# ShampooWang/SpeechCLIP_plus

Measured on AMD Instinct MI355X. Metric: utterances/sec (train step), higher is better.
Workload: dtype bf16; 1 GPU; Parallel SpeechCLIP base train step (HuBERT-base frozen fwd + weighted sum + CLS attention-pool head fwd/bwd + InfoNCE fwd/bwd + Adam), 64 utt/GPU x 10 s (L=160000, T=499), CLIP image embeddings given; global_batch=64, per_gpu_batch=64, audio_samples=160000, frames=499, parallelism=dp1

## Files before the change

speechclip_plus_amd/csrc/clspool.hip:

```cpp
#include "sc_common.h"

namespace {

constexpr int MAXH = 16;

template <int NH>
__device__ __forceinline__ float wave_sum_multi(float (&v)[NH], int lane, int& which) {
    int n = NH, off = 32;
    which = 0;
#pragma unroll
    for (int round = 0; round < 6; ++round) {
        if (n > 1) {
            const bool hi = (lane & off) != 0;
            const int half = n >> 1;
#pragma unroll
            for (int i = 0; i < NH / 2; ++i) {
                if (i < half) {
                    const float keep = hi ? v[i + half] : v[i];
                    const float send = hi ? v[i] : v[i + half];
                    v[i] = keep + __shfl_xor(send, off);
                }
            }
            which = which * 2 + (hi ? 1 : 0);
            n = half;
// ... 58 lines not shown
        }
    }
}

template <int NH>
__global__ __launch_bounds__(256) void cls_pool_fwd_kernel(const uint16_t* __restrict__ X,
                                                           const float* __restrict__ scores,
                                                           const int32_t* __restrict__ len, float* __restrict__ p,
                                                           float* __restrict__ m, int R, int D, int H,
                                                           const float* __restrict__ mult, float* __restrict__ psum) {
    extern __shared__ float sm[];
    float* ps = sm;
    float* red = sm + H * R;
    const int b = blockIdx.y, d0 = blockIdx.x * 64;
    const int lane = threadIdx.x & 63, wave = threadIdx.x >> 6;
    const int n = max(1, min(len[b], R));
    for (int h = wave; h < H; h += 4) {
        const float* sr = scores + ((int64_t)b * H + h) * R;
        float mx = -INFINITY;
        for (int s = lane; s < n; s += 64) mx = fmaxf(mx, sr[s]);
        mx = wave_max(mx);
        float sum = 0.f;
        for (int s = lane; s < n; s += 64) {
            const float e = __expf(sr[s] - mx);
            ps[h * R + s] = e;
            sum += e;
        }
        sum = wave_sum(sum);
        const float inv = 1.0f / sum;
        float kept = 0.f;
        for (int s = lane; s < R; s += 64) {
            const float v = s < n ? ps[h * R + s] * inv : 0.f;
            const float w = mult ? v * mult[((int64_t)b * H + h) * R + s] : v;
            ps[h * R + s] = w;
            kept += w;
            if (blockIdx.x == 0) p[((int64_t)b * H + h) * R + s] = v;
        }
        if (psum) {
            kept = wave_sum(kept);
            if (blockIdx.x == 0 && lane == 0) psum[(int64_t)b * H + h] = kept;
        }
    }
    __syncthreads();
    float acc[NH][8];
#pragma unroll
    for (int h = 0; h < NH; ++h)
#pragma unroll
        for (int e = 0; e < 8; ++e) acc[h][e] = 0.f;
    const int cchunk = lane & 7, rsub = lane >> 3;
    const uint16_t* xc = X + (int64_t)b * R * D + d0 + cchunk * 8;
    for (int s = wave * 8 + rsub; s < n; s += 32) {
        const uint4 u = *(const uint4*)(xc + (int64_t)s * D);
        const float x[8] = {bflo(u.x), bfhi(u.x), bflo(u.y), bfhi(u.y), bflo(u.z), bfhi(u.z), bflo(u.w), bfhi(u.w)};
#pragma unroll
        for (int h = 0; h < NH; ++h) {
            const float w = ps[h * R + s];
#pragma unroll
            for (int e = 0; e < 8; ++e) acc[h][e] = fmaf(w, x[e], acc[h][e]);
        }
    }
#pragma unroll
    for (int h = 0; h < NH; ++h)
#pragma unroll
        for (int e = 0; e < 8; ++e) {
            float v = acc[h][e];
            v += __shfl_xor(v, 8);
            v += __shfl_xor(v, 16);
            v += __shfl_xor(v, 32);
            if (rsub == 0) red[(wave * H + h) * 64 + cchunk * 8 + e] = v;
        }
    __syncthreads();
    for (int i = threadIdx.x; i < H * 64; i += 256) {
        const int h = i >> 6, d = i & 63;
        const float v = (red[(0 * H + h) * 64 + d] + red[(1 * H + h) * 64 + d]) +
                        (red[(2 * H + h) * 64 + d] + red[(3 * H + h) * 64 + d]);
        m[((int64_t)b * H + h) * D + d0 + d] = v;
    }
}

template <int NH>
__global__ __launch_bounds__(256) void cls_pool_bwd_kernel(const uint16_t* __restrict__ X,
                                                           const float* __restrict__ p,
                                                           const float* __restrict__ dp,
                                                           const float* __restrict__ dm,
                                                           const float* __restrict__ a,
                                                           const int32_t* __restrict__ len, float* __restrict__ dX,
                                                           float* __restrict__ da_partial, int R, int D, int H,
                                                           const float* __restrict__ mult, const float* __restrict__ cbias) {
    extern __shared__ float sm[];
    float* ps = sm;
    float* dss = sm + H * R;
    float* red = sm + 2 * H * R;
    const int b = blockIdx.y, d0 = blockIdx.x * 64;
    const int lane = threadIdx.x & 63, wave = threadIdx.x >> 6;
    const int n = max(1, min(len[b], R));
    for (int h = wave; h < H; h += 4) {
        const float* pr = p + ((int64_t)b * H + h) * R;
        const float* dpr = dp + ((int64_t)b * H + h) * R;
        const float* mr = mult ? mult + ((int64_t)b * H + h) * R : nullptr;
        const float cb = cbias ? cbias[(int64_t)b * H + h] : 0.f;
        auto dpe = [&](int s) { return cbias ? (dpr[s] + cb) * (mr ? mr[s] : 1.f) : dpr[s]; };
        float dot = 0.f;
        for (int s = lane; s < n; s += 64) dot += pr[s] * dpe(s);
        dot = wave_sum(dot);
        for (int s = lane; s < R; s += 64) {
            const float pv = s < n ? pr[s] : 0.f;
            ps[h * R + s] = mr ? pv * mr[s] : pv;
            dss[h * R + s] = s < n ? pv * (dpe(s) - dot) : 0.f;
        }
    }
    __syncthreads();
    const int cchunk = lane & 15, rsub = lane >> 4, c0 = d0 + cchunk * 4;
    f32x4 dmv[NH], av[NH], acc[NH];
#pragma unroll
    for (int h = 0; h < NH; ++h) {
        dmv[h] = *(const f32x4*)(dm + ((int64_t)b * H + h) * D + c0);
        av[h] = *(const f32x4*)(a + (int64_t)h * D + c0);
        acc[h] = f32x4{0.f, 0.f, 0.f, 0.f};
    }
    const uint16_t* xc = X + (int64_t)b * R * D + c0;
    float* gx = dX + (int64_t)b * R * D + c0;
    for (int s = wave * 4 + rsub; s < R; s += 16) {
        f32x4 g = {0.f, 0.f, 0.f, 0.f};
        if (s < n) {
            const uint2 u = *(const uint2*)(xc + (int64_t)s * D);
            const f32x4 x = {bflo(u.x), bfhi(u.x), bflo(u.y), bfhi(u.y)};
#pragma unroll
            for (int h = 0; h < NH; ++h) {
                const float dsv = dss[h * R + s], pw = ps[h * R + s];
                g += pw * dmv[h] + dsv * av[h];
                acc[h] += dsv * x;
            }
        }
        *(f32x4*)(gx + (int64_t)s * D) = g;
    }
#pragma unroll
    for (int h = 0; h < NH; ++h)
#pragma unroll
        for (int e = 0; e < 4; ++e) {
            float v = acc[h][e];
            v += __shfl_xor(v, 16);
            v += __shfl_xor(v, 32);
            if (rsub == 0) red[(wave * H + h) * 64 + cchunk * 4 + e] = v;
        }
    __syncthreads();
    for (int i = threadIdx.x; i < H * 64; i += 256) {
        const int h = i >> 6, d = i & 63;
        const float v = (red[(0 * H + h) * 64 + d] + red[(1 * H + h) * 64 + d]) +
                        (red[(2 * H + h) * 64 + d] + red[(3 * H + h) * 64 + d]);
        da_partial[((int64_t)b * H + h) * D + d0 + d] = v;
    }
}

}

extern "C" int sc_cls_scores(const sc_bf16* X, const float* vec, int64_t vec_bstride, float* scores, int32_t B,
                             int32_t R, int32_t D, int32_t H, void* stream) {
    SC_CHECK(X && vec && scores, "sc_cls_scores: null pointer");
    SC_CHECK(D % 4 == 0 && ((uintptr_t)X % 8) == 0 && ((uintptr_t)vec % 16) == 0 && vec_bstride % 4 == 0,
             "sc_cls_scores: alignment");
    SC_CHECK(D <= 1024, "sc_cls_scores: D=%d must be <= 1024", D);
    dim3 grid((R + 63) / 64, B);
    hipStream_t s = (hipStream_t)stream;
    const int nch = (D / 4 + 63) / 64;
#define SC_CS(NH, NC) hipLaunchKernelGGL((cls_scores_kernel<NH, NC>), grid, dim3(256), 0, s, X, vec, vec_bstride, scores, R, D, H, h0)
#define SC_CS_H(NH)                                                        \
    do {                                                                   \
        if (nch <= 1) SC_CS(NH, 1); else if (nch == 2) SC_CS(NH, 2); else if (nch == 3) SC_CS(NH, 3); else SC_CS(NH, 4); \
    } while (0)
    int h0 = 0;
    switch (H) {
        case 1: SC_CS_H(1); break;
        case 2: SC_CS_H(2); break;
        case 4: SC_CS_H(4); break;
        case 8: SC_CS_H(8); break;
        case 16:
            SC_CS_H(8);
            h0 = 8;
            SC_CS_H(8);
            break;
        default: sc_set_error("sc_cls_scores: H=%d not in {1,2,4,8,16}", H); return -1;
    }
#undef SC_CS_H
#undef SC_CS
    SC_LAUNCH_CHECK();
    return 0;
}

extern "C" int sc_cls_pool_fwd(const sc_bf16* X, const float* scores, const int32_t* len, float* p, float* m,
                               int32_t B, int32_t R, int32_t D, int32_t H, const float* mult, float* psum, void* stream) {
    SC_CHECK(X && scores && len && p && m, "sc_cls_pool_fwd: null pointer");
    SC_CHECK(D % 64 == 0 && H >= 1 && H <= MAXH && ((uintptr_t)X % 16) == 0, "sc_cls_pool_fwd: D %% 64, H <= 16, 16-byte aligned X required (D=%d H=%d)", D, H);
    const size_t lds = (size_t)(H * R + 4 * H * 64) * sizeof(float);
    SC_CHECK(lds <= 64 * 1024, "sc_cls_pool_fwd: H*R too large for LDS");
    #define SC_CPF(NH) hipLaunchKernelGGL(cls_pool_fwd_kernel<NH>, dim3(D / 64, B), dim3(256), lds, (hipStream_t)stream, X, scores, len, p, m, R, D, H, mult, psum)
    switch (H) {
        case 1: SC_CPF(1); break;
        case 2: SC_CPF(2); break;
        case 4: SC_CPF(4); break;
        case 8: SC_CPF(8); break;
        case 16: SC_CPF(16); break;
        default: sc_set_error("sc_cls_pool_fwd: H=%d not in {1,2,4,8,16}", H); return -1;
    }
#undef SC_CPF
    SC_LAUNCH_CHECK();
    return 0;
}

extern "C" int sc_cls_pool_bwd(const sc_bf16* X, const float* p, const float* dp, const float* dm, const float* a,
                               const int32_t* len, float* dX, float* da_partial, int32_t B, int32_t R, int32_t D,
                               int32_t H, const float* mult, const float* cbias, void* stream) {
    SC_CHECK(X && p && dp && dm && a && len && dX && da_partial, "sc_cls_pool_bwd: null pointer");
    SC_CHECK(D % 64 == 0 && H >= 1 && H <= MAXH, "sc_cls_pool_bwd: D %% 64, H <= 16 required");
    SC_CHECK(((uintptr_t)X % 8) == 0 && ((uintptr_t)dX % 16) == 0 && ((uintptr_t)dm % 16) == 0 && ((uintptr_t)a % 16) == 0, "sc_cls_pool_bwd: alignment");
    const size_t lds = (size_t)(2 * H * R + 4 * H * 64) * sizeof(float);
    SC_CHECK(lds <= 64 * 1024, "sc_cls_pool_bwd: H*R too large for LDS");
    #define SC_CPB(NH) hipLaunchKernelGGL(cls_pool_bwd_kernel<NH>, dim3(D / 64, B), dim3(256), lds, (hipStream_t)stream, X, p, dp, dm, a, len, dX, da_partial, R, D, H, mult, cbias)
    switch (H) {
        case 1: SC_CPB(1); break;
        case 2: SC_CPB(2); break;
        case 4: SC_CPB(4); break;
        case 8: SC_CPB(8); break;
        case 16: SC_CPB(16); break;
        default: sc_set_error("sc_cls_pool_bwd: H=%d not in {1,2,4,8,16}", H); return -1;
    }
#undef SC_CPB
    SC_LAUNCH_CHECK();
    return 0;
}
```

speechclip_plus_amd/csrc/rowops.hip:

```cpp
#include "sc_common.h"

namespace {

template <int NCH>
__global__ __launch_bounds__(256) void layernorm_kernel(const uint16_t* __restrict__ x, int64_t ldx,
                                                        const float* __restrict__ gamma,
                                                        const float* __restrict__ beta, uint16_t* __restrict__ y,
                                                        int64_t ldy, int64_t rows, int D, float eps, int act) {
    const int lane = threadIdx.x & 63;
    const int64_t row = (int64_t)blockIdx.x * 4 + (threadIdx.x >> 6);
    if (row >= rows) return;
    const int nchunks = D >> 2;
    float v[NCH][4];
    float sum = 0.f;
    const uint16_t* xr = x + row * ldx;
#pragma unroll
    for (int i = 0; i < NCH; ++i) {
        const int ch = lane + i * 64;
        if (ch < nchunks) {
            const uint2 u = *(const uint2*)(xr + ch * 4);
            v[i][0] = bflo(u.x); v[i][1] = bfhi(u.x); v[i][2] = bflo(u.y); v[i][3] = bfhi(u.y);
            sum += (v[i][0] + v[i][1]) + (v[i][2] + v[i][3]);
        } else {
            v[i][0] = v[i][1] = v[i][2] = v[i][3] = 0.f;
// ... 388 lines not shown
                load_row_norm<NE>(h + n * plane + m.src * D, lane, nchunks, D, 1e-5f, xh);
                const float wn = w[n];
#pragma unroll
                for (int i = 0; i < NE; ++i)
#pragma unroll
                    for (int j = 0; j < 8; ++j) acc[i][j] += wn * xh[i][j];
            }
        }
#pragma unroll
        for (int i = 0; i < NE; ++i) {
            const int ch = lane + i * 64;
            if (ch < nchunks) {
                uint4 o;
                o.x = pack2bf(acc[i][0], acc[i][1]); o.y = pack2bf(acc[i][2], acc[i][3]);
                o.z = pack2bf(acc[i][4], acc[i][5]); o.w = pack2bf(acc[i][6], acc[i][7]);
                *(uint4*)(out + m.out * D + ch * 8) = o;
            }
        }
    }
}

template <int NE, typename GT, typename Rows>
__global__ __launch_bounds__(256) void wsum_norm_bwd_kernel(const uint16_t* __restrict__ h, const GT* __restrict__ g, int NL,
                                                            float* __restrict__ dw_partial, Rows rows, int D, int row_off) {
    __shared__ float red[4][32];
    const int lane = threadIdx.x & 63, wave = threadIdx.x >> 6;
    const int nchunks = D >> 3;
    const int64_t count = rows.count(), plane = rows.plane(D);
    float accn[32];
#pragma unroll
    for (int n = 0; n < 32; ++n) accn[n] = 0.f;
    for (int64_t row = (int64_t)blockIdx.x * 4 + wave; row < count; row += (int64_t)gridDim.x * 4) {
        const RowRef m = rows.at(row, row_off);
        if (!m.live) continue;
        float gv[NE][8];
#pragma unroll
        for (int i = 0; i < NE; ++i) {
            const int ch = lane + i * 64;
            if (ch < nchunks) {
                f32x4 g0, g1;
                load_g8(g + m.out * D + ch * 8, g0, g1);
                gv[i][0] = g0[0]; gv[i][1] = g0[1]; gv[i][2] = g0[2]; gv[i][3] = g0[3];
                gv[i][4] = g1[0]; gv[i][5] = g1[1]; gv[i][6] = g1[2]; gv[i][7] = g1[3];
            } else {
#pragma unroll
                for (int j = 0; j < 8; ++j) gv[i][j] = 0.f;
            }
        }
        float xr[NE][8];
        load_row_norm<NE>(h + (int64_t)(NL - 1) * plane + m.src * D, lane, nchunks, D, 1e-5f, xr);
#pragma unroll
        for (int n = 0; n < 31; ++n) {
            if (n < NL - 1) {
                float xh[NE][8];
                load_row_norm<NE>(h + n * plane + m.src * D, lane, nchunks, D, 1e-5f, xh);
                float d = 0.f;
#pragma unroll
                for (int i = 0; i < NE; ++i)
#pragma unroll
                    for (int j = 0; j < 8; ++j) d += gv[i][j] * (xh[i][j] - xr[i][j]);
                accn[n] += d;
            }
        }
    }
#pragma unroll
    for (int n = 0; n < 32; ++n) {
        const float s = wave_sum(accn[n]);
        if (lane == 0) red[wave][n] = s;
    }
    __syncthreads();
    if (threadIdx.x < NL)
        dw_partial[(int64_t)blockIdx.x * NL + threadIdx.x] =
            (red[0][threadIdx.x] + red[1][threadIdx.x]) + (red[2][threadIdx.x] + red[3][threadIdx.x]);
}

__global__ __launch_bounds__(256) void posconv_prep_kernel(const uint16_t* __restrict__ x,
                                                           const int32_t* __restrict__ valid_len,
                                                           uint16_t* __restrict__ xz, uint16_t* __restrict__ xg,
                                                           int B, int R, int D, int G, int halo) {
    const int Dg = D / G;
    const int cpg = Dg >> 3;
    const int64_t chunks_per_row = D >> 3;
    const int64_t total = (int64_t)B * R * chunks_per_row;
    const int Rp = R + 2 * halo;
    for (int64_t q = (int64_t)blockIdx.x * blockDim.x + threadIdx.x; q < total; q += (int64_t)gridDim.x * blockDim.x) {
        const int64_t row = q / chunks_per_row;
        const int cc = (int)(q % chunks_per_row);
        const int b = (int)(row / R), t = (int)(row % R);
        uint4 u = make_uint4(0, 0, 0, 0);
        if (t < valid_len[b]) u = *(const uint4*)(x + row * D + cc * 8);
        *(uint4*)(xz + row * D + cc * 8) = u;
        const int g = cc / cpg, cg = cc % cpg;
        *(uint4*)(xg + (((int64_t)g * B + b) * Rp + halo + t) * Dg + cg * 8) = u;
    }
}


template <int NLT>
__global__ __launch_bounds__(256) void wsum_fwd_seg_fixed_kernel(const uint16_t* __restrict__ h, const float* __restrict__ w,
                                                                 uint16_t* __restrict__ out, const int32_t* __restrict__ row0, int Rout,
                                                                 int D, int row_off, int64_t plane) {
    const int cpr = D >> 3;
    const int idx = blockIdx.x * 256 + threadIdx.x;
    if (idx >= Rout * cpr) return;
    const int b = blockIdx.y;
    const int s = idx / cpr, cc = idx - s * cpr, t = s - row_off;
    const int r0 = row0[b], pitch = row0[b + 1] - r0;
    float acc[8] = {0, 0, 0, 0, 0, 0, 0, 0};
    if (t >= 0 && t < pitch) {
        const uint16_t* src = h + (int64_t)(r0 + t) * D + cc * 8;
        uint4 u[NLT];
#pragma unroll
        for (int n = 0; n < NLT; ++n) u[n] = *(const uint4*)(src + n * plane);
#pragma unroll
        for (int n = 0; n < NLT; ++n) {
            const float wn = w[n];
            acc[0] += wn * bflo(u[n].x); acc[1] += wn * bfhi(u[n].x); acc[2] += wn * bflo(u[n].y); acc[3] += wn * bfhi(u[n].y);
            acc[4] += wn * bflo(u[n].z); acc[5] += wn * bfhi(u[n].z); acc[6] += wn * bflo(u[n].w); acc[7] += wn * bfhi(u[n].w);
        }
    }
    uint4 o;
    o.x = pack2bf(acc[0], acc[1]); o.y = pack2bf(acc[2], acc[3]);
    o.z = pack2bf(acc[4], acc[5]); o.w = pack2bf(acc[6], acc[7]);
    *(uint4*)(out + ((int64_t)b * Rout + s) * D + cc * 8) = o;
}

template <int NLT, typename GT>
__global__ __launch_bounds__(256) void wsum_bwd_seg_fixed_kernel(const uint16_t* __restrict__ h, const GT* __restrict__ g,
                                                                 float* __restrict__ dw_partial, const int32_t* __restrict__ row0, int B, int Rout,
                                                                 int D, int row_off, int64_t plane) {
    __shared__ float red[4][32];
    const uint32_t cpr = (uint32_t)D >> 3, total = (uint32_t)B * (uint32_t)Rout * cpr, step = gridDim.x * 256u;
    float acc[NLT - 1];
#pragma unroll
    for (int n = 0; n < NLT - 1; ++n) acc[n] = 0.f;
    for (uint32_t q = blockIdx.x * 256u + threadIdx.x; q < total; q += step) {
        const uint32_t orow = q / cpr, cc = q - orow * cpr;
        const uint32_t b = orow / (uint32_t)Rout;
        const int t = (int)(orow - b * (uint32_t)Rout) - row_off;
        const int r0 = row0[b], pitch = row0[b + 1] - r0;
        if (t < 0 || t >= pitch) continue;
        f32x4 g0, g1;
        load_g8(g + (int64_t)orow * D + cc * 8, g0, g1);
        const uint16_t* src = h + (int64_t)(r0 + t) * D + cc * 8;
        const uint4 r = *(const uint4*)(src + (int64_t)(NLT - 1) * plane);
        uint4 u[NLT - 1];
#pragma unroll
        for (int n = 0; n < NLT - 1; ++n) u[n] = *(const uint4*)(src + n * plane);
#pragma unroll
        for (int n = 0; n < NLT - 1; ++n)
            acc[n] += g0[0] * (bflo(u[n].x) - bflo(r.x)) + g0[1] * (bfhi(u[n].x) - bfhi(r.x)) + g0[2] * (bflo(u[n].y) - bflo(r.y)) +
                      g0[3] * (bfhi(u[n].y) - bfhi(r.y)) + g1[0] * (bflo(u[n].z) - bflo(r.z)) + g1[1] * (bfhi(u[n].z) - bfhi(r.z)) +
                      g1[2] * (bflo(u[n].w) - bflo(r.w)) + g1[3] * (bfhi(u[n].w) - bfhi(r.w));
    }
    const int lane = threadIdx.x & 63, wave = threadIdx.x >> 6;
#pragma unroll
    for (int n = 0; n < NLT - 1; ++n) {
        const float sn = wave_sum(acc[n]);
        if (lane == 0) red[wave][n] = sn;
    }
    if (lane == 0) red[wave][NLT - 1] = 0.f;
    __syncthreads();
    if (threadIdx.x < NLT)
        dw_partial[(int64_t)blockIdx.x * NLT + threadIdx.x] =
            (red[0][threadIdx.x] + red[1][threadIdx.x]) + (red[2][threadIdx.x] + red[3][threadIdx.x]);
}

__global__ __launch_bounds__(256) void posconv_prep_seg_kernel(const uint16_t* __restrict__ x, const int32_t* __restrict__ valid_len,
                                                               uint16_t* __restrict__ xz, uint16_t* __restrict__ xg,
                                                               const int32_t* __restrict__ chunk, int rows, int B, int D, int G, int halo) {
    const int Dg = D / G;
    const int cpg = Dg >> 3;
    const int64_t chunks_per_row = D >> 3;
    const int64_t total = (int64_t)rows * chunks_per_row;
    const int64_t slab_rows = (int64_t)rows + 2 * halo * B;
    for (int64_t q = (int64_t)blockIdx.x * blockDim.x + threadIdx.x; q < total; q += (int64_t)gridDim.x * blockDim.x) {
        const int row = (int)(q / chunks_per_row);
        const int cc = (int)(q % chunks_per_row);
        const int4 sg = *(const int4*)(chunk + 4 * (row >> 3));
        const int t = row - sg.x, pitch = sg.y, b = sg.z;
        uint4 u = make_uint4(0, 0, 0, 0);
        if (t < valid_len[b]) u = *(const uint4*)(x + (int64_t)row * D + cc * 8);
        *(uint4*)(xz + (int64_t)row * D + cc * 8) = u;
        const int g = cc / cpg, cg = cc % cpg;
        uint16_t* slab = xg + ((int64_t)g * slab_rows + sg.x + 2 * halo * b) * Dg + cg * 8;
        *(uint4*)(slab + (int64_t)(halo + t) * Dg) = u;
        const uint4 z = make_uint4(0, 0, 0, 0);
        for (int v = t; v < halo; v += pitch) {
            *(uint4*)(slab + (int64_t)v * Dg) = z;
            *(uint4*)(slab + (int64_t)(halo + pitch + v) * Dg) = z;
        }
    }
}

}

extern "C" int sc_layernorm_bf16(const sc_bf16* x, int64_t ldx, const float* gamma, const float* beta, sc_bf16* y,
                                 int64_t ldy, int64_t rows, int32_t D, float eps, int32_t act, void* stream) {
    SC_CHECK(x && gamma && beta && y, "sc_layernorm_bf16: null pointer");
    SC_CHECK(D > 0 && D % 4 == 0 && D <= 1024, "sc_layernorm_bf16: D=%d must be a multiple of 4, <= 1024", D);
    SC_CHECK(ldx % 4 == 0 && ldy % 4 == 0 && rows > 0, "sc_layernorm_bf16: bad ld/rows");
    SC_CHECK(((uintptr_t)x % 8) == 0 && ((uintptr_t)y % 8) == 0 && ((uintptr_t)gamma % 16) == 0 &&
                 ((uintptr_t)beta % 16) == 0, "sc_layernorm_bf16: alignment");
    hipStream_t s = (hipStream_t)stream;
    if (D % 8 == 0 && ldx % 8 == 0 && ldy % 8 == 0 && ((uintptr_t)x % 16) == 0 && ((uintptr_t)y % 16) == 0) {
        dim3 grid8((unsigned)((rows + 7) / 8));
        const int nch8 = (D / 8 + 31) / 32;
        if (nch8 <= 2) hipLaunchKernelGGL(layernorm16_kernel<2>, grid8, dim3(256), 0, s, x, ldx, gamma, beta, y, ldy, rows, D, eps, act);
        else if (nch8 == 3) hipLaunchKernelGGL(layernorm16_kernel<3>, grid8, dim3(256), 0, s, x, ldx, gamma, beta, y, ldy, rows, D, eps, act);
        else hipLaunchKernelGGL(layernorm16_kernel<4>, grid8, dim3(256), 0, s, x, ldx, gamma, beta, y, ldy, rows, D, eps, act);
        SC_LAUNCH_CHECK();
        return 0;
    }
    dim3 grid((unsigned)((rows + 3) / 4));
    const int nch = (D / 4 + 63) / 64;
    if (nch <= 2) hipLaunchKernelGGL(layernorm_kernel<2>, grid, dim3(256), 0, s, x, ldx, gamma, beta, y, ldy, rows, D, eps, act);
    else if (nch == 3) hipLaunchKernelGGL(layernorm_kernel<3>, grid, dim3(256), 0, s, x, ldx, gamma, beta, y, ldy, rows, D, eps, act);
    else hipLaunchKernelGGL(layernorm_kernel<4>, grid, dim3(256), 0, s, x, ldx, gamma, beta, y, ldy, rows, D, eps, act);
    SC_LAUNCH_CHECK();
    return 0;
}

namespace {

template <typename Rows>
int wsum_fwd_launch(const uint16_t* h, const float* w, int NL, uint16_t* out, const Rows& rows, int D, int row_off, bool normalize, int grid,
                    hipStream_t s) {
    if (!normalize) hipLaunchKernelGGL(wsum_fwd_kernel<Rows>, dim3(grid), dim3(256), 0, s, h, w, NL, out, rows, D, row_off);
    else if (D <= 512) hipLaunchKernelGGL((wsum_norm_fwd_kernel<1, Rows>), dim3(grid), dim3(256), 0, s, h, w, NL, out, rows, D, row_off);
    else hipLaunchKernelGGL((wsum_norm_fwd_kernel<2, Rows>), dim3(grid), dim3(256), 0, s, h, w, NL, out, rows, D, row_off);
    SC_LAUNCH_CHECK();
    return 0;
}

template <typename Rows>
int wsum_bwd_launch(const uint16_t* h, const void* gv, int NL, float* dw_partial, int nblk, const Rows& rows, int D, int row_off, int flags,
                    hipStream_t s) {
    const bool normalize = flags & 1, g16 = flags & 2;
    const float* g = (const float*)gv;
    const uint16_t* gh = (const uint16_t*)gv;
    if (!normalize) {
        if (g16) hipLaunchKernelGGL((wsum_bwd_kernel<uint16_t, Rows>), dim3(nblk), dim3(256), 0, s, h, gh, NL, dw_partial, rows, D, row_off);
        else hipLaunchKernelGGL((wsum_bwd_kernel<float, Rows>), dim3(nblk), dim3(256), 0, s, h, g, NL, dw_partial, rows, D, row_off);
    } else if (D <= 512) {
        if (g16) hipLaunchKernelGGL((wsum_norm_bwd_kernel<1, uint16_t, Rows>), dim3(nblk), dim3(256), 0, s, h, gh, NL, dw_partial, rows, D, row_off);
        else hipLaunchKernelGGL((wsum_norm_bwd_kernel<1, float, Rows>), dim3(nblk), dim3(256), 0, s, h, g, NL, dw_partial, rows, D, row_off);
    } else {
        if (g16) hipLaunchKernelGGL((wsum_norm_bwd_kernel<2, uint16_t, Rows>), dim3(nblk), dim3(256), 0, s, h, gh, NL, dw_partial, rows, D, row_off);
        else hipLaunchKernelGGL((wsum_norm_bwd_kernel<2, float, Rows>), dim3(nblk), dim3(256), 0, s, h, g, NL, dw_partial, rows, D, row_off);
    }
    SC_LAUNCH_CHECK();
    return 0;
}

template int wsum_fwd_launch(const uint16_t*, const float*, int, uint16_t*, const UniformRows&, int, int, bool, int, hipStream_t);
template int wsum_bwd_launch(const uint16_t*, const void*, int, float*, int, const UniformRows&, int, int, int, hipStream_t);

}

extern "C" int sc_wsum_fwd(const sc_bf16* h, const float* w, int32_t NL, sc_bf16* out, const sc_segments* seg, int32_t B, int32_t R,
                           int32_t D, int32_t row_off, int32_t normalize, void* stream) {
    SC_CHECK(h && w && out && (!seg || seg->row0), "sc_wsum_fwd: null pointer");
    SC_CHECK(NL >= 1 && NL <= 32 && D % 8 == 0 && row_off >= 0 && row_off < R && (!seg || (seg->B > 0 && seg->rows > 0)), "sc_wsum_fwd: bad NL/D/row_off");
    SC_CHECK(!seg || B == seg->B, "sc_wsum_fwd: B=%d against seg->B=%d", B, seg->B);
    if (normalize) SC_CHECK(D <= 1024, "sc_wsum_fwd: normalised variant needs D <= 1024 (got %d)", D);
    hipStream_t s = (hipStream_t)stream;
    const int64_t plane = seg ? (int64_t)seg->rows * D : 0;
    if (seg && !normalize && (NL == 13 || NL == 25) && (int64_t)R * (D / 8) < (1ll << 30) && B <= 65535 && !sc_option(5)) {
        const dim3 g2((unsigned)(((int64_t)R * (D / 8) + 255) / 256), (unsigned)B);
        if (NL == 13) hipLaunchKernelGGL(wsum_fwd_seg_fixed_kernel<13>, g2, dim3(256), 0, s, h, w, out, seg->row0, R, D, row_off, plane);
        else hipLaunchKernelGGL(wsum_fwd_seg_fixed_kernel<25>, g2, dim3(256), 0, s, h, w, out, seg->row0, R, D, row_off, plane);
        SC_LAUNCH_CHECK();
        return 0;
    }
    const int64_t rows = (int64_t)B * R, total = rows * (D / 8);
    const int grid = normalize ? (int)((rows + 3) / 4 < 4096 ? (rows + 3) / 4 : 4096) : (int)((total + 255) / 256 < 2048 ? (total + 255) / 256 : 2048);
    return seg ? wsum_fwd_launch(h, w, NL, out, SegRows{seg->row0, B, R, plane}, D, row_off, normalize, grid, s)
               : wsum_fwd_launch(h, w, NL, out, UniformRows{B, R}, D, row_off, normalize, grid, s);
}

extern "C" int sc_wsum_bwd(const sc_bf16* h, const void* gv, int32_t NL, float* dw_partial, int32_t nblk, const sc_segments* seg, int32_t B,
                           int32_t R, int32_t D, int32_t row_off, int32_t flags, void* stream) {
    SC_CHECK(h && gv && dw_partial && (!seg || seg->row0), "sc_wsum_bwd: null pointer");
    SC_CHECK(((uintptr_t)gv % 16) == 0, "sc_wsum_bwd: g must be 16-byte aligned");
    const bool normalize = flags & 1, g16 = flags & 2;
    SC_CHECK(NL >= 1 && NL <= 32 && D % 8 == 0 && nblk >= 1 && row_off >= 0 && row_off < R && (!seg || (seg->B > 0 && seg->rows > 0)), "sc_wsum_bwd: bad args");
    SC_CHECK(!seg || B == seg->B, "sc_wsum_bwd: B=%d against seg->B=%d", B, seg->B);
    if (normalize) SC_CHECK(D <= 1024, "sc_wsum_bwd: normalised variant needs D <= 1024 (got %d)", D);
    hipStream_t s = (hipStream_t)stream;
    if (!seg) return wsum_bwd_launch(h, gv, NL, dw_partial, nblk, UniformRows{B, R}, D, row_off, flags, s);
    const int64_t plane = (int64_t)seg->rows * D;
    if (!normalize && (NL == 13 || NL == 25) && (int64_t)B * R * (D / 8) < (1ll << 31) && !sc_option(5)) {
        const float* g = (const float*)gv;
        const uint16_t* gh = (const uint16_t*)gv;
        if (NL == 13) {
            if (g16) hipLaunchKernelGGL((wsum_bwd_seg_fixed_kernel<13, uint16_t>), dim3(nblk), dim3(256), 0, s, h, gh, dw_partial, seg->row0, B, R, D, row_off, plane);
            else hipLaunchKernelGGL((wsum_bwd_seg_fixed_kernel<13, float>), dim3(nblk), dim3(256), 0, s, h, g, dw_partial, seg->row0, B, R, D, row_off, plane);
        } else {
            if (g16) hipLaunchKernelGGL((wsum_bwd_seg_fixed_kernel<25, uint16_t>), dim3(nblk), dim3(256), 0, s, h, gh, dw_partial, seg->row0, B, R, D, row_off, plane);
            else hipLaunchKernelGGL((wsum_bwd_seg_fixed_kernel<25, float>), dim3(nblk), dim3(256), 0, s, h, g, dw_partial, seg->row0, B, R, D, row_off, plane);
        }
        SC_LAUNCH_CHECK();
        return 0;
    }
    return wsum_bwd_launch(h, gv, NL, dw_partial, nblk, SegRows{seg->row0, B, R, plane}, D, row_off, flags, s);
}

extern "C" int sc_wsum_lazy_fwd(const sc_bf16* h, const float* w, int32_t NL, sc_bf16* out, int32_t B, int32_t R, int32_t D,
                                int32_t row_off, const float* stats, const float* gamma, const float* beta, int32_t first_lazy,
                                int32_t ns, float eps, void* stream) {
    SC_CHECK(h && w && out && stats && gamma && beta, "sc_wsum_lazy_fwd: null pointer");
    SC_CHECK(NL >= 1 && NL <= 32 && D % 8 == 0 && row_off >= 0 && row_off < R && ns >= 1 && ns <= 8 && first_lazy >= 0 && eps > 0.f,
             "sc_wsum_lazy_fwd: bad NL / D / row_off / strips");
    const LazyLn z{stats, gamma, beta, first_lazy, ns, eps};
    const int64_t total = (int64_t)B * R * (D / 8);
    const int grid = (int)((total + 255) / 256 < 2048 ? (total + 255) / 256 : 2048);
    hipLaunchKernelGGL(wsum_lazy_fwd_kernel, dim3(grid), dim3(256), 0, (hipStream_t)stream, h, w, NL, out, B, R, D, row_off, z);
    SC_LAUNCH_CHECK();
    return 0;
}

extern "C" int sc_wsum_lazy_bwd(const sc_bf16* h, const float* g, int32_t NL, float* dw_partial, int32_t nblk, int32_t B, int32_t R,
                                int32_t D, int32_t row_off, const float* stats, const float* gamma, const float* beta,
                                int32_t first_lazy, int32_t ns, float eps, void* stream) {
    SC_CHECK(h && g && dw_partial && stats && gamma && beta, "sc_wsum_lazy_bwd: null pointer");
    SC_CHECK(NL >= 1 && NL <= 32 && D % 8 == 0 && nblk >= 1 && row_off >= 0 && row_off < R && ns >= 1 && ns <= 8 && eps > 0.f,
             "sc_wsum_lazy_bwd: bad args");
    const LazyLn z{stats, gamma, beta, first_lazy, ns, eps};
    hipLaunchKernelGGL(wsum_lazy_bwd_kernel, dim3(nblk), dim3(256), 0, (hipStream_t)stream, h, g, NL, dw_partial, B, R, D, row_off, z);
    SC_LAUNCH_CHECK();
    return 0;
}

extern "C" int sc_posconv_prep(const sc_bf16* x, const int32_t* valid_len, sc_bf16* xz, sc_bf16* xg, const sc_segments* seg, int32_t B,
                               int32_t R, int32_t D, int32_t G, int32_t halo, void* stream) {
    SC_CHECK(x && valid_len && xz && xg && (!seg || seg->chunk), "sc_posconv_prep: null pointer");
    if (seg) {
        SC_CHECK(G > 0 && D % G == 0 && (D / G) % 8 == 0 && seg->rows > 0 && seg->rows % SC_SEG_ROWS == 0 && seg->B > 0 && halo > 0,
                 "sc_posconv_prep: D/G=%d must be a multiple of 8, rows a multiple of 8", D / G);
        SC_CHECK(((uintptr_t)seg->chunk % 16) == 0, "sc_posconv_prep: chunk table must be 16-byte aligned");
    } else {
        SC_CHECK(G > 0 && D % G == 0 && (D / G) % 8 == 0, "sc_posconv_prep: D/G=%d must be a multiple of 8", D / G);
    }
    const int64_t total = (seg ? (int64_t)seg->rows : (int64_t)B * R) * (D / 8);
    const int grid = (int)((total + 255) / 256 < 4096 ? (total + 255) / 256 : 4096);
    if (seg)
        hipLaunchKernelGGL(posconv_prep_seg_kernel, dim3(grid), dim3(256), 0, (hipStream_t)stream, x, valid_len, xz, xg, seg->chunk, seg->rows, seg->B, D, G, halo);
    else
        hipLaunchKernelGGL(posconv_prep_kernel, dim3(grid), dim3(256), 0, (hipStream_t)stream, x, valid_len, xz, xg, B, R, D, G, halo);
    SC_LAUNCH_CHECK();
    return 0;
}
```

Baseline: 5641 utterances/s.

## Add hand-scheduled variants of CLS pooling and layer weighted-sum kernels

Adds new variants of the CLS score, pooling forward and backward kernels and of the segmented weighted-sum forward and backward kernels, selected by default unless option 4 is set. The new kernels use 32-bit offsets, scalar base pointers, LDS-staged weight tables, two rows per iteration and asm register ties that force load and FMA ordering, while reproducing the original kernels' rounding order. The aim is lower address arithmetic, better memory-level parallelism and fewer wasted loads in these bandwidth-bound passes. This adds a large amount of fragile code that depends on specific head and layer counts and on exact compiler rounding behaviour.

```diff
diff --git a/speechclip_plus_amd/csrc/clspool.hip b/speechclip_plus_amd/csrc/clspool.hip
--- a/speechclip_plus_amd/csrc/clspool.hip
+++ b/speechclip_plus_amd/csrc/clspool.hip
@@ -234,6 +234,315 @@
     }
 }
 
+
+
+__device__ __forceinline__ float dot4(int first, float x0, float x1, float x2, float x3, const f32x4& v) {
+#pragma clang fp contract(off)
+    float t = first ? x1 * v[1] : x0 * v[0];
+    t = first ? fmaf(x0, v[0], t) : fmaf(x1, v[1], t);
+    t = fmaf(x2, v[2], t);
+    return fmaf(x3, v[3], t);
+}
+
+template <int NH>
+__device__ __forceinline__ float wave_sum_multi_late(float (&v)[NH], int lane, int& which) {
+    auto shfl_xor = [&](float x, int off) { return __int_as_float(__builtin_amdgcn_ds_bpermute((lane ^ off) << 2, __float_as_int(x))); };
+    int n = NH, off = 32;
+    which = 0;
+#pragma unroll
+    for (int round = 0; round < 6; ++round) {
+        if (n > 1) {
+            const bool hi = (lane & off) != 0;
+            const int half = n >> 1;
+#pragma unroll
+            for (int i = 0; i < NH / 2; ++i) {
+                if (i < half) {
+                    const float keep = hi ? v[i + half] : v[i];
+                    const float send = hi ? v[i] : v[i + half];
+                    v[i] = keep + shfl_xor(send, off);
+                }
+            }
+            which = which * 2 + (hi ? 1 : 0);
+            n = half;
+        } else {
+            v[0] += shfl_xor(v[0], off);
+        }
+        off >>= 1;
+    }
+    return v[0];
+}
+
+template <int NH, int NCH>
+__global__ __launch_bounds__(256) void cls_scores_co_kernel(const uint16_t* __restrict__ X, const float* __restrict__ vec, int64_t vec_bstride,
+                                                            float* __restrict__ scores, int R, int Htot, int h0) {
+    constexpr int D = 256 * NCH;
+    const int b = blockIdx.y;
+    const int lane = threadIdx.x & 63, wave = threadIdx.x >> 6;
+    const float* vb = vec + (int64_t)b * vec_bstride + (int64_t)h0 * D;
+    __shared__ f32x4 vs[NH * 64 * NCH];
+    for (int i = threadIdx.x; i < NH * 64 * NCH; i += 256) vs[i] = *(const f32x4*)(vb + (int64_t)i * 4);
+    __syncthreads();
+    constexpr int ROWS = 64, RPW = ROWS / 4;
+    static_assert(NH == 8, "dot4's table of roundings is the 8-head kernels'");
+    constexpr unsigned kMulFirst1 = NCH == 1 ? 0xaau : 0x56u;
+    const int s0 = blockIdx.x * ROWS + wave * RPW;
+    const char* xb = (const char*)X + (int64_t)b * R * D * 2;
+#pragma unroll 1
+    for (int g = 0; g < RPW; g += 2) {
+        int vo = lane;
+        asm volatile("" : "+v"(vo));
+        uint2 u0[NCH], u1[NCH];
+        {
+            const uint32_t o0 = (uint32_t)min(s0 + g, R - 1) * (uint32_t)(D * 2) + (uint32_t)vo * 8u;
+            const uint32_t o1 = (uint32_t)min(s0 + g + 1, R - 1) * (uint32_t)(D * 2) + (uint32_t)vo * 8u;
+#pragma unroll
+            for (int c = 0; c < NCH; ++c) {
+                u0[c] = *(const uint2*)(xb + o0 + 512 * c);
+                u1[c] = *(const uint2*)(xb + o1 + 512 * c);
+            }
+        }
+        float acc0[NH], acc1[NH];
+#pragma unroll
+        for (int h = 0; h < NH; ++h) acc0[h] = acc1[h] = 0.f;
+#pragma unroll
+        for (int c = 0; c < NCH; ++c) {
+            if (c > 0) asm("" : "+v"(u0[c].x), "+v"(u0[c].y), "+v"(u1[c].x), "+v"(u1[c].y) : "v"(acc0[NH - 1]), "v"(acc1[NH - 1]));
+            const float x0 = bflo(u0[c].x), x1 = bfhi(u0[c].x), x2 = bflo(u0[c].y), x3 = bfhi(u0[c].y);
+            const float y0 = bflo(u1[c].x), y1 = bfhi(u1[c].x), y2 = bflo(u1[c].y), y3 = bfhi(u1[c].y);
+#pragma unroll
+            for (int h = 0; h < NH; ++h) {
+                int vk = vo;
+                const int k2 = c * NH + h - 2;
+                if (k2 >= 0) asm("" : "+v"(vk) : "v"(acc0[k2 % NH]), "v"(acc1[k2 % NH]));
+                const f32x4 v = vs[h * (64 * NCH) + 64 * c + vk];
+                acc0[h] += dot4((kMulFirst1 >> h) & 1, x0, x1, x2, x3, v);
+                acc1[h] += dot4((kMulFirst1 >> h) & 1, y0, y1, y2, y3, v);
+            }
+        }
+        constexpr int LOWMASK = 63 >> 3;
+        int h, ln = vo;
+        asm volatile("" : "+v"(ln) : "v"(acc0[NH - 1]), "v"(acc1[NH - 1]));
+        const float t0 = wave_sum_multi_late<NH>(acc0, ln, h);
+        if ((ln & LOWMASK) == 0 && s0 + g < R) scores[((int64_t)b * Htot + h0 + h) * R + s0 + g] = t0;
+        const float t1 = wave_sum_multi_late<NH>(acc1, ln, h);
+        if ((ln & LOWMASK) == 0 && s0 + g + 1 < R) scores[((int64_t)b * Htot + h0 + h) * R + s0 + g + 1] = t1;
+    }
+}
+
+template <int NH>
+__global__ __launch_bounds__(256) void cls_pool_fwd_co_kernel(const uint16_t* __restrict__ X, const float* __restrict__ scores,
+                                                              const int32_t* __restrict__ len, float* __restrict__ p, float* __restrict__ m, int R,
+                                                              int D, int H, const float* __restrict__ mult, float* __restrict__ psum) {
+    extern __shared__ float sm[];
+    float* ps = sm;
+    float* red = sm + H * R;
+    const int b = blockIdx.y, d0 = blockIdx.x * 64;
+    const int lane = threadIdx.x & 63, wave = threadIdx.x >> 6;
+    const int n = max(1, min(len[b], R));
+    for (int h = wave; h < H; h += 4) {
+        const float* sr = scores + ((int64_t)b * H + h) * R;
+        float mx = -INFINITY;
+        for (int s = lane; s < n; s += 64) mx = fmaxf(mx, sr[s]);
+        mx = wave_max(mx);
+        float sum = 0.f;
+        for (int s = lane; s < n; s += 64) {
+            const float e = __expf(sr[s] - mx);
+            ps[h * R + s] = e;
+            sum += e;
+        }
+        sum = wave_sum(sum);
+        const float inv = 1.0f / sum;
+        float kept = 0.f;
+        for (int s = lane; s < R; s += 64) {
+            const float v = s < n ? ps[h * R + s] * inv : 0.f;
+            const float w = mult ? v * mult[((int64_t)b * H + h) * R + s] : v;
+            ps[h * R + s] = w;
+            kept += w;
+            if (blockIdx.x == 0) p[((int64_t)b * H + h) * R + s] = v;
+        }
+        if (psum) {
+            kept = wave_sum(kept);
+            if (blockIdx.x == 0 && lane == 0) psum[(int64_t)b * H + h] = kept;
+        }
+    }
+    __syncthreads();
+    constexpr int HG = NH <= 4 ? NH : NH / 2;
+    const int cchunk = lane & 7, rsub = lane >> 3;
+    const uint16_t* xc = X + (int64_t)b * R * D + d0 + cchunk * 8;
+#pragma unroll 1
+    for (int hg = 0; hg < NH; hg += HG) {
+        float acc[HG][8];
+#pragma unroll
+        for (int h = 0; h < HG; ++h)
+#pragma unroll
+            for (int e = 0; e < 8; ++e) acc[h][e] = 0.f;
+        const float* pg = ps + hg * R;
+#pragma unroll 1
+        for (int s = wave * 8 + rsub; s < n; s += 32) {
+            const uint4 u = *(const uint4*)(xc + (int64_t)s * D);
+            const float x[8] = {bflo(u.x), bfhi(u.x), bflo(u.y), bfhi(u.y), bflo(u.z), bfhi(u.z), bflo(u.w), bfhi(u.w)};
+#pragma unroll
+            for (int h = 0; h < HG; ++h) {
+                int sw = s;
+                if (h > 0) asm("" : "+v"(sw) : "v"(acc[h - 1][7]));
+                const float w = pg[h * R + sw];
+#pragma unroll
+                for (int e = 0; e < 8; ++e) acc[h][e] = fmaf(w, x[e], acc[h][e]);
+            }
+        }
+#pragma unroll
+        for (int h = 0; h < HG; ++h)
+#pragma unroll
+            for (int e = 0; e < 8; ++e) {
+                float v = acc[h][e];
+                v += __shfl_xor(v, 8);
+                v += __shfl_xor(v, 16);
+                v += __shfl_xor(v, 32);
+                if (rsub == 0) red[(wave * H + hg + h) * 64 + cchunk * 8 + e] = v;
+            }
+    }
+    __syncthreads();
+    for (int i = threadIdx.x; i < H * 64; i += 256) {
+        const int h = i >> 6, d = i & 63;
+        const float v = (red[(0 * H + h) * 64 + d] + red[(1 * H + h) * 64 + d]) +
+                        (red[(2 * H + h) * 64 + d] + red[(3 * H + h) * 64 + d]);
+        m[((int64_t)b * H + h) * D + d0 + d] = v;
+    }
+}
+
+template <typename T>
+__device__ __forceinline__ T* uniform_ptr(T* p) {
+    const uint64_t v = (uint64_t)p;
+    const uint32_t lo = __builtin_amdgcn_readfirstlane((uint32_t)v), hi = __builtin_amdgcn_readfirstlane((uint32_t)(v >> 32));
+    return (T*)(((uint64_t)hi << 32) | lo);
+}
+
+template <int NH>
+__global__ __launch_bounds__(256) void cls_pool_bwd_co_kernel(const uint16_t* __restrict__ X, const float* __restrict__ p,
+                                                              const float* __restrict__ dp, const float* __restrict__ dm,
+                                                              const float* __restrict__ a, const int32_t* __restrict__ len,
+                                                              float* __restrict__ dX, float* __restrict__ da_partial, int R, int D, int H,
+                                                              const float* __restrict__ mult, const float* __restrict__ cbias) {
+#pragma clang fp contract(off)
+    static_assert(NH == 8, "the roundings spelled out below are those of cls_pool_bwd_kernel<8> as compiled");
+    constexpr int TS = 128;
+    __shared__ f32x4 dms[NH][16], as[NH][16];
+    __shared__ f32x2 wt[NH][TS];
+    __shared__ float red[4 * NH * 64];
+    __shared__ float dots[NH];
+    const int b = blockIdx.y, d0 = blockIdx.x * 64;
+    const int lane = threadIdx.x & 63, wave = threadIdx.x >> 6;
+    const int n = max(1, min(len[b], R));
+    const int uwave = __builtin_amdgcn_readfirstlane(wave);
+    auto dpe = [&](const float* dpr, const float* mr, float cb, int s) { return cbias ? (dpr[s] + cb) * (mr ? mr[s] : 1.f) : dpr[s]; };
+    for (int h = uwave; h < NH; h += 4) {
+        const float* pr = p + ((int64_t)b * H + h) * R;
+        const float* dpr = dp + ((int64_t)b * H + h) * R;
+        const float* mr = mult ? mult + ((int64_t)b * H + h) * R : nullptr;
+        const float cb = cbias ? cbias[(int64_t)b * H + h] : 0.f;
+        float dot = 0.f;
+        for (int s = lane; s < n; s += 64) dot = fmaf(pr[s], dpe(dpr, mr, cb, s), dot);
+        dot = wave_sum(dot);
+        if (lane == 0) dots[h] = dot;
+    }
+    for (int i = threadIdx.x; i < NH * 16; i += 256) {
+        const int h = i >> 4, cq = i & 15;
+        dms[h][cq] = *(const f32x4*)(dm + (uint32_t)((b * H + h) * D + d0 + cq * 4));
+        as[h][cq] = *(const f32x4*)(a + (uint32_t)(h * D + d0 + cq * 4));
+    }
+    f32x4 acc[NH];
+#pragma unroll
+    for (int h = 0; h < NH; ++h)
+#pragma unroll
+        for (int e = 0; e < 4; ++e) {
+            float z = 0.f;
+            asm volatile("" : "+v"(z));
+            acc[h][e] = z;
+        }
+    const char* xb = (const char*)X + (int64_t)b * R * D * 2;
+    char* gb = (char*)dX + (int64_t)b * R * D * 4;
+    xb = uniform_ptr(xb);
+    gb = uniform_ptr(gb);
+    typedef uint32_t u32x2 __attribute__((ext_vector_type(2)));
+#pragma unroll 1
+    for (int t0 = 0; t0 < R; t0 += TS) {
+        const int t1 = min(R, t0 + TS);
+        __syncthreads();
+        for (int h = uwave; h < NH; h += 4) {
+            const float* pr = p + ((int64_t)b * H + h) * R;
+            const float* dpr = dp + ((int64_t)b * H + h) * R;
+            const float* mr = mult ? mult + ((int64_t)b * H + h) * R : nullptr;
+            const float cb = cbias ? cbias[(int64_t)b * H + h] : 0.f;
+            const float dot = dots[h];
+            int fl = threadIdx.x;
+            asm volatile("" : "+v"(fl));
+            for (int s = t0 + (fl & 63); s < t1; s += 64) {
+                const float pv = s < n ? pr[s] : 0.f;
+                f32x2 t;
+                t.x = mr ? pv * mr[s] : pv;
+                t.y = s < n ? pv * (dpe(dpr, mr, cb, s) - dot) : 0.f;
+                wt[h][s - t0] = t;
+            }
+        }
+        __syncthreads();
+        int tid = threadIdx.x;
+        asm volatile("" : "+v"(tid));
+        const int cq0 = tid & 15, co0 = d0 + cq0 * 4;
+#pragma unroll 1
+        for (int s = t0 + (tid >> 4); s < t1; s += 16) {
+            f32x4 g = {0.f, 0.f, 0.f, 0.f};
+            if (s < n) {
+                int cq = cq0;
+                asm volatile("" : "+v"(cq));
+                const u32x2 u = *(const __attribute__((address_space(1))) u32x2*)((const __attribute__((address_space(1))) char*)xb + ((uint32_t)s * (uint32_t)D + (uint32_t)co0) * 2u);
+                const f32x4 x = {bflo(u.x), bfhi(u.x), bflo(u.y), bfhi(u.y)};
+                float tie1 = 0.f, tie1b = 0.f;
+#pragma unroll
+                for (int h = 0; h < NH; ++h) {
+                    int ch = cq, sh = s - t0;
+                    if (h >= 1) asm("" : "+v"(ch), "+v"(sh) : "v"(tie1), "v"(tie1b), "v"(acc[h - 1][1]), "v"(acc[h - 1][3]));
+                    else asm("" : "+v"(ch), "+v"(sh) : "v"(x[1]), "v"(x[3]));
+                    const f32x2 t = wt[h][sh];
+                    const float dsv = t.y, pw = t.x;
+#pragma unroll
+                    for (int e2 = 0; e2 < 2; ++e2) {
+                        const int ce = 2 * ch + e2;
+                        const f32x2 dmh = ((const f32x2*)&dms[h][0])[ce], ah = ((const f32x2*)&as[h][0])[ce];
+#pragma unroll
+                        for (int j = 0; j < 2; ++j) {
+                            const int e = 2 * e2 + j;
+                            g[e] = g[e] + fmaf(dsv, ah[j], pw * dmh[j]);
+                            acc[h][e] = fmaf(dsv, x[e], acc[h][e]);
+                        }
+                    }
+                    tie1 = g[0]; tie1b = g[3];
+                }
+            }
+            *(__attribute__((address_space(1))) f32x4*)((__attribute__((address_space(1))) char*)gb + ((uint32_t)s * (uint32_t)D + (uint32_t)co0) * 4u) = g;
+        }
+    }
+    int tl = threadIdx.x;
+    asm volatile("" : "+v"(tl));
+    const int cchunk_l = tl & 15, rsub_l = (tl >> 4) & 3, wave_l = tl >> 6;
+    auto shfl_xor_l = [&](float x, int off) { return __int_as_float(__builtin_amdgcn_ds_bpermute(((tl & 63) ^ off) << 2, __float_as_int(x))); };
+#pragma unroll
+    for (int h = 0; h < NH; ++h)
+#pragma unroll
+        for (int e = 0; e < 4; ++e) {
+            float v = acc[h][e];
+            v += shfl_xor_l(v, 16);
+            v += shfl_xor_l(v, 32);
+            if (rsub_l == 0) red[(wave_l * NH + h) * 64 + cchunk_l * 4 + e] = v;
+        }
+    __syncthreads();
+    for (int i = threadIdx.x; i < NH * 64; i += 256) {
+        const int h = i >> 6, d = i & 63;
+        const float v = (red[(0 * NH + h) * 64 + d] + red[(1 * NH + h) * 64 + d]) +
+                        (red[(2 * NH + h) * 64 + d] + red[(3 * NH + h) * 64 + d]);
+        da_partial[(uint32_t)((b * H + h) * D + d0 + d)] = v;
+    }
+}
+
 }
 
 extern "C" int sc_cls_scores(const sc_bf16* X, const float* vec, int64_t vec_bstride, float* scores, int32_t B,
@@ -245,7 +554,12 @@
     dim3 grid((R + 63) / 64, B);
     hipStream_t s = (hipStream_t)stream;
     const int nch = (D / 4 + 63) / 64;
-#define SC_CS(NH, NC) hipLaunchKernelGGL((cls_scores_kernel<NH, NC>), grid, dim3(256), 0, s, X, vec, vec_bstride, scores, R, D, H, h0)
+    const bool co = !sc_option(4) && (int64_t)R * D < (1ll << 31);
+#define SC_CS(NH, NC)                                                                                                               \
+    do {                                                                                                                            \
+        if (co && NH == 8 && D == 256 * NC) hipLaunchKernelGGL((cls_scores_co_kernel<8, NC>), grid, dim3(256), 0, s, X, vec, vec_bstride, scores, R, H, h0); \
+        else hipLaunchKernelGGL((cls_scores_kernel<NH, NC>), grid, dim3(256), 0, s, X, vec, vec_bstride, scores, R, D, H, h0);      \
+    } while (0)
 #define SC_CS_H(NH)                                                        \
     do {                                                                   \
         if (nch <= 1) SC_CS(NH, 1); else if (nch == 2) SC_CS(NH, 2); else if (nch == 3) SC_CS(NH, 3); else SC_CS(NH, 4); \
@@ -275,7 +589,12 @@
     SC_CHECK(D % 64 == 0 && H >= 1 && H <= MAXH && ((uintptr_t)X % 16) == 0, "sc_cls_pool_fwd: D %% 64, H <= 16, 16-byte aligned X required (D=%d H=%d)", D, H);
     const size_t lds = (size_t)(H * R + 4 * H * 64) * sizeof(float);
     SC_CHECK(lds <= 64 * 1024, "sc_cls_pool_fwd: H*R too large for LDS");
-    #define SC_CPF(NH) hipLaunchKernelGGL(cls_pool_fwd_kernel<NH>, dim3(D / 64, B), dim3(256), lds, (hipStream_t)stream, X, scores, len, p, m, R, D, H, mult, psum)
+    const bool co = !sc_option(4);
+    #define SC_CPF(NH)                                                                                                                                      \
+    do {                                                                                                                                                    \
+        if (co) hipLaunchKernelGGL(cls_pool_fwd_co_kernel<NH>, dim3(D / 64, B), dim3(256), lds, (hipStream_t)stream, X, scores, len, p, m, R, D, H, mult, psum); \
+        else hipLaunchKernelGGL(cls_pool_fwd_kernel<NH>, dim3(D / 64, B), dim3(256), lds, (hipStream_t)stream, X, scores, len, p, m, R, D, H, mult, psum);      \
+    } while (0)
     switch (H) {
         case 1: SC_CPF(1); break;
         case 2: SC_CPF(2); break;
@@ -297,7 +616,12 @@
     SC_CHECK(((uintptr_t)X % 8) == 0 && ((uintptr_t)dX % 16) == 0 && ((uintptr_t)dm % 16) == 0 && ((uintptr_t)a % 16) == 0, "sc_cls_pool_bwd: alignment");
     const size_t lds = (size_t)(2 * H * R + 4 * H * 64) * sizeof(float);
     SC_CHECK(lds <= 64 * 1024, "sc_cls_pool_bwd: H*R too large for LDS");
-    #define SC_CPB(NH) hipLaunchKernelGGL(cls_pool_bwd_kernel<NH>, dim3(D / 64, B), dim3(256), lds, (hipStream_t)stream, X, p, dp, dm, a, len, dX, da_partial, R, D, H, mult, cbias)
+    const bool co = !sc_option(4) && (int64_t)R * D < (1ll << 30) && (int64_t)B * H * D < (1ll << 31);
+    #define SC_CPB(NH)                                                                                                                                                         \
+    do {                                                                                                                                                                       \
+        if (co && NH == 8) hipLaunchKernelGGL(cls_pool_bwd_co_kernel<8>, dim3(D / 64, B), dim3(256), 0, (hipStream_t)stream, X, p, dp, dm, a, len, dX, da_partial, R, D, H, mult, cbias); \
+        else hipLaunchKernelGGL(cls_pool_bwd_kernel<NH>, dim3(D / 64, B), dim3(256), lds, (hipStream_t)stream, X, p, dp, dm, a, len, dX, da_partial, R, D, H, mult, cbias);    \
+    } while (0)
     switch (H) {
         case 1: SC_CPB(1); break;
         case 2: SC_CPB(2); break;
diff --git a/speechclip_plus_amd/csrc/rowops.hip b/speechclip_plus_amd/csrc/rowops.hip
--- a/speechclip_plus_amd/csrc/rowops.hip
+++ b/speechclip_plus_amd/csrc/rowops.hip
@@ -564,6 +564,117 @@
             acc[n] += g0[0] * (bflo(u[n].x) - bflo(r.x)) + g0[1] * (bfhi(u[n].x) - bfhi(r.x)) + g0[2] * (bflo(u[n].y) - bflo(r.y)) +
                       g0[3] * (bfhi(u[n].y) - bfhi(r.y)) + g1[0] * (bflo(u[n].z) - bflo(r.z)) + g1[1] * (bfhi(u[n].z) - bfhi(r.z)) +
                       g1[2] * (bflo(u[n].w) - bflo(r.w)) + g1[3] * (bfhi(u[n].w) - bfhi(r.w));
+    }
+    const int lane = threadIdx.x & 63, wave = threadIdx.x >> 6;
+#pragma unroll
+    for (int n = 0; n < NLT - 1; ++n) {
+        const float sn = wave_sum(acc[n]);
+        if (lane == 0) red[wave][n] = sn;
+    }
+    if (lane == 0) red[wave][NLT - 1] = 0.f;
+    __syncthreads();
+    if (threadIdx.x < NLT)
+        dw_partial[(int64_t)blockIdx.x * NLT + threadIdx.x] =
+            (red[0][threadIdx.x] + red[1][threadIdx.x]) + (red[2][threadIdx.x] + red[3][threadIdx.x]);
+}
+
+
+typedef uint32_t u32x4 __attribute__((ext_vector_type(4)));
+__device__ __forceinline__ uint4 load_layer16(const char* hb, int n, int64_t plane, uint32_t off) {
+    const char* p = hb + n * plane * 2;
+    asm("" : "+s"(p));
+    const u32x4 v = *(const __attribute__((address_space(1))) u32x4*)((const __attribute__((address_space(1))) char*)p + off);
+    return make_uint4(v.x, v.y, v.z, v.w);
+}
+
+template <int NLT>
+__global__ __launch_bounds__(256) void wsum_fwd_seg_fixed_co_kernel(const uint16_t* __restrict__ h, const float* __restrict__ w,
+                                                                       uint16_t* __restrict__ out, const int32_t* __restrict__ row0, int Rout,
+                                                                       int D, int row_off, int64_t plane) {
+    const int cpr = D >> 3;
+    const int idx = blockIdx.x * 256 + threadIdx.x;
+    if (idx >= Rout * cpr) return;
+    const int b = blockIdx.y;
+    const int s = idx / cpr, cc = idx - s * cpr, t = s - row_off;
+    const int r0 = row0[b], pitch = row0[b + 1] - r0;
+    float acc[8] = {0, 0, 0, 0, 0, 0, 0, 0};
+    if (t >= 0 && t < pitch) {
+        const uint32_t off = ((uint32_t)(r0 + t) * (uint32_t)D + (uint32_t)cc * 8u) * 2u;
+        const char* hb = (const char*)h;
+        uint4 u[NLT];
+#pragma unroll
+        for (int n = 0; n < NLT; ++n) u[n] = load_layer16(hb, n, plane, off);
+#pragma unroll
+        for (int n = 0; n < NLT; ++n) {
+            const float wn = w[n];
+            if (n > 0) asm("" : "+v"(u[n].x), "+v"(u[n].y), "+v"(u[n].z), "+v"(u[n].w) : "v"(acc[0]), "v"(acc[7]));
+            acc[0] = fmaf(wn, bflo(u[n].x), acc[0]); acc[1] = fmaf(wn, bfhi(u[n].x), acc[1]);
+            acc[2] = fmaf(wn, bflo(u[n].y), acc[2]); acc[3] = fmaf(wn, bfhi(u[n].y), acc[3]);
+            acc[4] = fmaf(wn, bflo(u[n].z), acc[4]); acc[5] = fmaf(wn, bfhi(u[n].z), acc[5]);
+            acc[6] = fmaf(wn, bflo(u[n].w), acc[6]); acc[7] = fmaf(wn, bfhi(u[n].w), acc[7]);
+        }
+    }
+    uint4 o;
+    o.x = pack2bf(acc[0], acc[1]); o.y = pack2bf(acc[2], acc[3]);
+    o.z = pack2bf(acc[4], acc[5]); o.w = pack2bf(acc[6], acc[7]);
+    const uint32_t oo = (((uint32_t)b * (uint32_t)Rout + (uint32_t)s) * (uint32_t)D + (uint32_t)cc * 8u) * 2u;
+    *(uint4*)((char*)out + oo) = o;
+}
+
+template <int NLT>
+__device__ __forceinline__ float layer_dot(int n, const f32x4& g0, const f32x4& g1, const uint4& u, const uint4& r) {
+#pragma clang fp contract(off)
+    static_assert(NLT == 13, "the table of roundings below is the 13-layer kernel's");
+    const float g[8] = {g0[0], g0[1], g0[2], g0[3], g1[0], g1[1], g1[2], g1[3]};
+    const float d[8] = {bflo(u.x) - bflo(r.x), bfhi(u.x) - bfhi(r.x), bflo(u.y) - bflo(r.y), bfhi(u.y) - bfhi(r.y),
+                        bflo(u.z) - bflo(r.z), bfhi(u.z) - bfhi(r.z), bflo(u.w) - bflo(r.w), bfhi(u.w) - bfhi(r.w)};
+    float t;
+    if (n >= 10) {
+        t = g[0] * d[0] + g[1] * d[1];
+#pragma unroll
+        for (int k = 2; k < 8; ++k) t = t + g[k] * d[k];
+        return t;
+    }
+    const int first = n & 1;
+    t = g[first] * d[first];
+    t = fmaf(g[first ^ 1], d[first ^ 1], t);
+#pragma unroll
+    for (int k = 2; k < 8; ++k) t = fmaf(g[k], d[k], t);
+    return t;
+}
+
+template <int NLT, int GRP, typename GT>
+__global__ __launch_bounds__(256) void wsum_bwd_seg_fixed_co_kernel(const uint16_t* __restrict__ h, const GT* __restrict__ g,
+                                                                       float* __restrict__ dw_partial, const int32_t* __restrict__ row0, int B,
+                                                                       int Rout, int D, int row_off, int64_t plane) {
+    static_assert((NLT - 1) % GRP == 0, "the groups cover the layers exactly");
+    __shared__ float red[4][32];
+    const uint32_t cpr = (uint32_t)D >> 3, total = (uint32_t)B * (uint32_t)Rout * cpr, step = gridDim.x * 256u;
+    const char* hb = (const char*)h;
+    float acc[NLT - 1];
+#pragma unroll
+    for (int n = 0; n < NLT - 1; ++n) acc[n] = 0.f;
+    for (uint32_t q = blockIdx.x * 256u + threadIdx.x; q < total; q += step) {
+        const uint32_t orow = q / cpr, cc = q - orow * cpr;
+        const uint32_t b = orow / (uint32_t)Rout;
+        const int t = (int)(orow - b * (uint32_t)Rout) - row_off;
+        const int r0 = row0[b], pitch = row0[b + 1] - r0;
+        if (t < 0 || t >= pitch) continue;
+        f32x4 g0, g1;
+        load_g8((const GT*)((const char*)g + q * (uint32_t)(8 * sizeof(GT))), g0, g1);
+        const uint32_t off = ((uint32_t)(r0 + t) * (uint32_t)D + cc * 8u) * 2u;
+        const uint4 r = load_layer16(hb, NLT - 1, plane, off);
+#pragma unroll
+        for (int n0 = 0; n0 < NLT - 1; n0 += GRP) {
+            uint4 u[GRP];
+#pragma unroll
+            for (int i = 0; i < GRP; ++i) u[i] = load_layer16(hb, n0 + i, plane, off);
+#pragma unroll
+            for (int i = 0; i < GRP; ++i) {
+                if (n0 + i > 0) asm("" : "+v"(u[i].x), "+v"(u[i].y), "+v"(u[i].z), "+v"(u[i].w) : "v"(acc[n0 + i - 1]));
+                acc[n0 + i] += layer_dot<NLT>(n0 + i, g0, g1, u[i], r);
+            }
+        }
     }
     const int lane = threadIdx.x & 63, wave = threadIdx.x >> 6;
 #pragma unroll
@@ -680,7 +791,9 @@
     const int64_t plane = seg ? (int64_t)seg->rows * D : 0;
     if (seg && !normalize && (NL == 13 || NL == 25) && (int64_t)R * (D / 8) < (1ll << 30) && B <= 65535 && !sc_option(5)) {
         const dim3 g2((unsigned)(((int64_t)R * (D / 8) + 255) / 256), (unsigned)B);
-        if (NL == 13) hipLaunchKernelGGL(wsum_fwd_seg_fixed_kernel<13>, g2, dim3(256), 0, s, h, w, out, seg->row0, R, D, row_off, plane);
+        const bool co = NL == 13 && plane * 2 < (1ll << 32) && (int64_t)B * R * D * 2 < (1ll << 32) && !sc_option(4);
+        if (co) hipLaunchKernelGGL(wsum_fwd_seg_fixed_co_kernel<13>, g2, dim3(256), 0, s, h, w, out, seg->row0, R, D, row_off, plane);
+        else if (NL == 13) hipLaunchKernelGGL(wsum_fwd_seg_fixed_kernel<13>, g2, dim3(256), 0, s, h, w, out, seg->row0, R, D, row_off, plane);
         else hipLaunchKernelGGL(wsum_fwd_seg_fixed_kernel<25>, g2, dim3(256), 0, s, h, w, out, seg->row0, R, D, row_off, plane);
         SC_LAUNCH_CHECK();
         return 0;
@@ -705,7 +818,10 @@
     if (!normalize && (NL == 13 || NL == 25) && (int64_t)B * R * (D / 8) < (1ll << 31) && !sc_option(5)) {
         const float* g = (const float*)gv;
         const uint16_t* gh = (const uint16_t*)gv;
-        if (NL == 13) {
+        const bool co = NL == 13 && !g16 && plane * 2 < (1ll << 32) && (int64_t)B * R * D * 4 < (1ll << 32) && !sc_option(4);
+        if (co) {
+            hipLaunchKernelGGL((wsum_bwd_seg_fixed_co_kernel<13, 4, float>), dim3(nblk), dim3(256), 0, s, h, g, dw_partial, seg->row0, B, R, D, row_off, plane);
+        } else if (NL == 13) {
             if (g16) hipLaunchKernelGGL((wsum_bwd_seg_fixed_kernel<13, uint16_t>), dim3(nblk), dim3(256), 0, s, h, gh, dw_partial, seg->row0, B, R, D, row_off, plane);
             else hipLaunchKernelGGL((wsum_bwd_seg_fixed_kernel<13, float>), dim3(nblk), dim3(256), 0, s, h, g, dw_partial, seg->row0, B, R, D, row_off, plane);
         } else {
```

After: 5662 utterances/s, median of 4. No clear change (+0.4%).
